# generalizable-neural-performer/bodyfitting

Measured on NVIDIA B200. Metric: fitted frames/s (SMPL-X, 8 views, 100 iters), higher is better.
Workload: dtype fp32

## Files before the change

bodyfitting_b200/csrc/bf_api.cu:

```cuda
#include <math.h>
#include <stdarg.h>
#include <string.h>
#include <stddef.h>
#include <stdlib.h>

#include "bf_common.cuh"
#include "bf_pose.cuh"
#include "bf_skin.cuh"
#include "bf_loss.cuh"
#include "bf_gmm.cuh"
#include "bf_frame.cuh"
#include "bf_ops.cuh"
#include "bf_grid.cuh"
#include "bf_mask.cuh"
#include "../../include/bodyfit_b200_ops.h"
#include "bf_blend_tc.cuh"
#include "bf_blend_tc2.cuh"
#include "bf_pack.cuh"
#include "bf_model_build.cuh"

static thread_local char g_err[512] = "";

void bf_set_error(const char* fmt, ...) {
    va_list ap;
    va_start(ap, fmt);
    vsnprintf(g_err, sizeof(g_err), fmt, ap);
    va_end(ap);
}

static int check_model(const BfModel* m, const BfFrames* f) {
    BF_REQUIRE(m && f, "null model / frames");
    BF_REQUIRE(m->J > 0 && m->J <= BF_MAXJ, "J out of range");
    BF_REQUIRE(m->NS > 0 && m->NS <= BF_MAXNS && m->NB <= m->NS, "NS/NB out of range");
    BF_REQUIRE(m->face == 0 || (m->face == 1 && m->is_smplx), "face parameters apply to SMPL-X only");
    BF_REQUIRE(m->NP == theta_layout(*m).np && theta_layout(m->is_smplx, m->NB).np <= BF_MAXNP && m->NP <= BF_THETA_SMEM,
               "NP does not match theta layout");
    BF_REQUIRE(m->Kp % 16 == 0 && m->Kp >= m->P + m->NS + 1, "Kp must be a multiple of 16 covering P+NS+1");
    BF_REQUIRE(m->P == (m->J - 1) * 9, "P != 9(J-1)");
    BF_REQUIRE(m->parents && m->lvl_ptr && m->lvl_j && m->child_ptr && m->child_idx, "kinematic tree tables missing");
    BF_REQUIRE(f->B > 0, "B <= 0");
    BF_REQUIRE(f->theta, "theta is null");
    return BF_OK;
}

static int check_vset(const BfVSet* vs, const BfFrames* f) {
    BF_REQUIRE(vs->Bm && vs->ell_j && vs->ell_w, "vertex set tables missing");
    BF_REQUIRE(vs->n > 0 && vs->n_pad % 32 == 0 && vs->n_pad >= vs->n && vs->ldn == 3 * vs->n_pad, "bad vertex set padding");
    BF_REQUIRE(f->ld_v >= 3 * vs->n, "ld_v < 3n");
    BF_REQUIRE(vs->K_out <= BF_MAXK, "too many output joints");
    return BF_OK;
}

extern "C" {

int bf_abi_version(void) { return BF_ABI_VERSION; }
int bf_sizeof(int which) {
    switch (which) {
        case 0: return (int)sizeof(BfVSet);
        case 1: return (int)sizeof(BfModel);
        case 2: return (int)sizeof(BfFrames);
        case 3: return (int)sizeof(BfGrid);
        case 4: return (int)sizeof(BfSmpld);
        case 5: return (int)sizeof(BfMask);
        default: return -1;
    }
}
const char* bf_last_error(void) { return g_err; }

int bf_check_device(void) {
    int dev = 0;
    cudaDeviceProp p;
    if (cudaGetDevice(&dev) != cudaSuccess || cudaGetDeviceProperties(&p, dev) != cudaSuccess) {
        bf_set_error("bf_check_device: no CUDA device");
        return BF_ECUDA;
    }
    if (p.major != 10) {
        bf_set_error("bf_check_device: device %s is sm_%d%d; this library is sm_100a only (no fallback)", p.name, p.major, p.minor);
        return BF_EARCH;
    }
    return BF_OK;
}

int bf_pose_forward(const BfModel* m, const BfFrames* f, void* stream) {
    BF_NVTX();
    int rc = check_model(m, f); if (rc) return rc;
    BF_REQUIRE(f->pf && f->A && f->Jtr, "pf/A/Jtr is null");
    const int wpb = 4;
    const dim3 grid((f->B + wpb - 1) / wpb), block(32 * wpb);
    k_pose_fwd<<<grid, block, wpb * sizeof(PoseSmem), (cudaStream_t)stream>>>(*m, *f);
    BF_LAUNCH_CHECK();
    return BF_OK;
}

int bf_skin_forward(const BfModel* m, const BfFrames* f, int use_full, void* stream) {
    BF_NVTX();
    int rc = check_model(m, f); if (rc) return rc;
    const BfVSet* vs = use_full ? &m->full : &m->act;
    rc = check_vset(vs, f); if (rc) return rc;
    BF_REQUIRE(f->pf && f->A && f->verts, "pf/A/verts is null");
    if (bf_tc_ready_fwd(vs, f)) {
        float* vp = f->vposed ? f->vposed : f->verts;
        rc = bf_blend_forward_tc(m, vs, f, vp, (cudaStream_t)stream); if (rc) return rc;
        rc = bf_launch_skin_frame(0, m, vs, f, vp, f->verts, nullptr, nullptr, 0, (f->flags & BF_F_WORLD) ? 1 : 0, 0, (cudaStream_t)stream);
        if (rc != 1) return rc;
        return bf_launch_skin_rows(0, vs, m->J, f->A, vp, f->verts, nullptr, nullptr, f->B, f->ld_v, 0,
                                   (f->flags & BF_F_WORLD) ? f->theta : nullptr, m->NP, f->constant_scale, (cudaStream_t)stream);
    }
    const dim3 grid(vs->n_pad / SK_TV, (f->B + SK_TB - 1) / SK_TB), block(256);
    k_skin_fwd<<<grid, block, 0, (cudaStream_t)stream>>>(*vs, m->J, m->Kp, f->pf, f->A, f->verts, f->vposed, f->B, f->ld_v,
                                                           (f->flags & BF_F_WORLD) ? f->theta : nullptr, m->NP, f->constant_scale);
    BF_LAUNCH_CHECK();
    return BF_OK;
}

int bf_blend_forward(const BfModel* m, const BfFrames* f, int use_full, void* stream) {
    BF_NVTX();
    int rc = check_model(m, f); if (rc) return rc;
    const BfVSet* vs = use_full ? &m->full : &m->act;
    rc = check_vset(vs, f); if (rc) return rc;
    BF_REQUIRE(f->vposed, "vposed is null");
    BF_REQUIRE((f->flags & BF_F_TC) && vs->Bt_hi && vs->Bt_lo && f->pf_hi && f->pf_lo, "bf_blend_forward needs the tensor-core operands (BF_F_TC)");
    return bf_blend_forward_tc(m, vs, f, f->vposed, (cudaStream_t)stream);
}

int bf_joints_forward(const BfModel* m, const BfFrames* f, int use_full, void* stream) {
    BF_NVTX();
    int rc = check_model(m, f); if (rc) return rc;
    const BfVSet* vs = use_full ? &m->full : &m->act;
    rc = check_vset(vs, f); if (rc) return rc;
    BF_REQUIRE(f->joints && f->Jtr && f->verts, "joints/Jtr/verts is null");
    k_joints_fwd<<<f->B, 160, 0, (cudaStream_t)stream>>>(*m, *vs, *f);
    BF_LAUNCH_CHECK();
    return BF_OK;
}

int bf_joints_backward(const BfModel* m, const BfFrames* f, int use_full, int accumulate_dverts, void* stream) {
    BF_NVTX();
    int rc = check_model(m, f); if (rc) return rc;
    const BfVSet* vs = use_full ? &m->full : &m->act;
    rc = check_vset(vs, f); if (rc) return rc;
    BF_REQUIRE(f->dJtr && f->dverts, "dJtr/dverts is null");
    k_joints_bwd<<<f->B, 256, 0, (cudaStream_t)stream>>>(*m, *vs, *f, accumulate_dverts);
    BF_LAUNCH_CHECK();
    return BF_OK;
}

int bf_keypoint_loss(const BfModel* m, const BfFrames* f, int use_full, void* stream) {
    BF_NVTX();
    int rc = check_model(m, f); if (rc) return rc;
    const BfVSet* vs = use_full ? &m->full : &m->act;
    rc = check_vset(vs, f); if (rc) return rc;
    BF_REQUIRE(f->kp && f->cams && f->loss && f->grad && f->dJtr && f->dverts && f->verts && f->Jtr, "loss buffers missing");
    BF_REQUIRE(f->Nv > 0 && f->Nv <= BF_MAXVIEWS, "Nv out of range");
    BF_REQUIRE(m->K_used <= vs->K_out, "K_used > K_out");
    const int threads = use_full ? 256 : 160;
    k_keypoint_loss<<<f->B, threads, 0, (cudaStream_t)stream>>>(*m, *vs, *f);
    BF_LAUNCH_CHECK();
    return BF_OK;
}

struct SideStream { cudaStream_t main = nullptr; cudaStream_t s = nullptr; cudaEvent_t fork = nullptr, join = nullptr; int dev = -1, slot = 0; };
static SideStream* side_stream(cudaStream_t main_s, int slot = 0) {
    static SideStream table[512];
    static int used = 0;
    int dev = 0;
    if (cudaGetDevice(&dev) != cudaSuccess) return nullptr;
    std::lock_guard<std::mutex> lk(g_bf_mu);
    for (int i = 0; i < used; ++i)
        if (table[i].dev == dev && table[i].main == main_s && table[i].slot == slot) return &table[i];
    if (used >= 512) return nullptr;
    SideStream* ss = &table[used];
    if (cudaStreamCreateWithFlags(&ss->s, cudaStreamNonBlocking) != cudaSuccess) return nullptr;
// ... 128 lines not shown
        rc = bf_gemm_forward_tc(x_hi, x_lo, m->gmm_bt_hi, m->gmm_bt_lo, f->B, GM_KG, ny, ny / 3, Y, ny, s); if (rc) return rc;
        k_gmm_select<<<(f->B + 3) / 4, 128, 0, s>>>(*m, f->theta + 7, m->NP, nb, f->B, Y, ny, wp, f->gmm_grad, f->gmm_loss);
        BF_LAUNCH_CHECK();
        return BF_OK;
    }
    return launch_gmm(m, f->theta + 7, m->NP, theta_layout(m->is_smplx).nbody, f->B, f->w_pose * f->w_pose,
                      f->gmm_grad, f->gmm_loss, (cudaStream_t)stream);
}

int bf_op_project(const float* pts, const float* R, const float* t, const float* K, float* uv, int B, int N, int nb, void* stream) {
    BF_REQUIRE(pts && R && t && K && uv && B > 0 && N > 0 && (nb == 1 || nb == B), "bad arguments");
    k_project_fwd<<<(B * N + 255) / 256, 256, 0, (cudaStream_t)stream>>>(pts, R, t, K, uv, B, N, nb);
    BF_LAUNCH_CHECK();
    return BF_OK;
}
int bf_op_project_backward(const float* pts, const float* R, const float* t, const float* K, const float* duv, float* dpts,
                           int B, int N, int nb, void* stream) {
    BF_REQUIRE(pts && R && t && K && duv && dpts && B > 0 && N > 0 && (nb == 1 || nb == B), "bad arguments");
    k_project_bwd<<<(B * N + 255) / 256, 256, 0, (cudaStream_t)stream>>>(pts, R, t, K, duv, dpts, B, N, nb);
    BF_LAUNCH_CHECK();
    return BF_OK;
}
int bf_op_gmof(const float* x, float* y, float sigma, int64_t n, void* stream) {
    BF_REQUIRE(x && y && n > 0, "bad arguments");
    k_gmof_fwd<<<(unsigned)((n + 255) / 256), 256, 0, (cudaStream_t)stream>>>(x, y, sigma, (size_t)n);
    BF_LAUNCH_CHECK();
    return BF_OK;
}
int bf_op_gmof_backward(const float* x, const float* dy, float* dx, float sigma, int64_t n, void* stream) {
    BF_REQUIRE(x && dy && dx && n > 0, "bad arguments");
    k_gmof_bwd<<<(unsigned)((n + 255) / 256), 256, 0, (cudaStream_t)stream>>>(x, dy, dx, sigma, (size_t)n);
    BF_LAUNCH_CHECK();
    return BF_OK;
}
int bf_op_reprojection(const float* cord, const float* gt, const float* w, float coef, float sigma, int N, float* out,
                       float* dcord, void* stream) {
    BF_REQUIRE(cord && gt && w && out && dcord && N > 0, "bad arguments");
    k_reproj<<<1, 256, 0, (cudaStream_t)stream>>>(cord, gt, w, coef, sigma, N, out, dcord);
    BF_LAUNCH_CHECK();
    return BF_OK;
}
int bf_op_keypoints_world(const float* joints, const float* kp, const float* cams, int B, int K, int Nv, float coef,
                          float sigma, float* loss_bk, float* dJ, void* stream) {
    BF_REQUIRE(joints && kp && cams && loss_bk && dJ && B > 0 && K > 0 && Nv > 0, "bad arguments");
    k_kp_world<<<(B * K + 127) / 128, 128, 0, (cudaStream_t)stream>>>(joints, kp, cams, B, K, Nv, coef, sigma, loss_bk, dJ);
    BF_LAUNCH_CHECK();
    return BF_OK;
}
int bf_op_angle_prior(const float* pose, int B, int D, float* out, float* dout, void* stream) {
    BF_REQUIRE(pose && out && dout && B > 0 && D >= 56, "bad arguments (pose needs >= 56 columns)");
    k_angle_prior<<<(B * 4 + 127) / 128, 128, 0, (cudaStream_t)stream>>>(pose, B, D, out, dout);
    BF_LAUNCH_CHECK();
    return BF_OK;
}
int bf_op_gmm_pose(const BfModel* m, const float* pose, int ld, int nvalid, int B, float weight, float* grad, float* loss,
                   void* stream) {
    BF_REQUIRE(m && nvalid > 0 && nvalid <= 69 && ld >= nvalid, "bad arguments");
    return launch_gmm(m, pose, ld, nvalid, B, weight, grad, loss, (cudaStream_t)stream);
}

int bf_pose_backward(const BfModel* m, const BfFrames* f, int flags, void* stream) {
    BF_NVTX();
    int rc = check_model(m, f); if (rc) return rc;
    BF_REQUIRE(f->dA && f->dJtr && f->dpf && f->grad && f->loss, "pose backward buffers missing");
    if (flags & 1) BF_REQUIRE(f->gmm_grad && f->gmm_loss, "gmm_grad / gmm_loss missing (run bf_gmm_prior first)");
    if (flags & 8) BF_REQUIRE((flags & 2) && f->pf && f->A && f->Jtr, "flag 8 needs the Adam step and the forward buffers");
    if (flags & 2) BF_REQUIRE(f->adam_m && f->adam_v, "Adam state missing");
    const double t = (double)(f->iter + 1);
    const double bc1 = 1.0 - pow(f->beta1, t);
    const double bc2 = 1.0 - pow(f->beta2, t);
    AdamArgs ad;
    ad.step_ts = (float)(f->lr_ts / bc1);
    ad.step_lr = (float)(f->lr / bc1);
    ad.bc2_sqrt = (float)sqrt(bc2);
    ad.beta2 = (float)f->beta2;
    ad.om_beta1 = (float)(1.0 - f->beta1);
    ad.om_beta2 = (float)(1.0 - f->beta2);
    ad.eps = (float)f->eps;
    static int wpb = 0;
    if (!wpb) { const char* e = getenv("BODYFIT_POSE_WPB"); wpb = e ? atoi(e) : 2; if (wpb < 1 || wpb > 4) wpb = 2; }
    const dim3 grid((f->B + wpb - 1) / wpb), block(32 * wpb);
    BfFrames g = *f;
    if (!bf_bwd_two_cta(m, f)) g.dpf2 = nullptr;
    k_pose_bwd<<<grid, block, wpb * sizeof(PoseSmemBwd), (cudaStream_t)stream>>>(*m, g, flags, ad);
    BF_LAUNCH_CHECK();
    return BF_OK;
}

int bf_lbs_forward(const BfModel* m, const BfFrames* f, void* stream) {
    BF_NVTX();
    int rc = bf_pose_forward(m, f, stream); if (rc) return rc;
    const BfVSet* vs = &m->full;
    if (f->joints && bf_tc_ready_fwd(vs, f) && f->verts && f->Jtr) {
        rc = check_vset(vs, f); if (rc) return rc;
        float* vp = f->vposed ? f->vposed : f->verts;
        rc = bf_blend_forward_tc(m, vs, f, vp, (cudaStream_t)stream); if (rc) return rc;
        rc = bf_launch_skin_frame(0, m, vs, f, vp, f->verts, nullptr, nullptr, 0, (f->flags & BF_F_WORLD) ? 1 : 0, 1, (cudaStream_t)stream);
        if (rc == 2) return BF_OK;
        if (rc == BF_OK) return bf_joints_forward(m, f, 1, stream);
        if (rc != 1) return rc;
        rc = bf_launch_skin_rows(0, vs, m->J, f->A, vp, f->verts, nullptr, nullptr, f->B, f->ld_v, 0,
                                 (f->flags & BF_F_WORLD) ? f->theta : nullptr, m->NP, f->constant_scale, (cudaStream_t)stream);
        if (rc) return rc;
        return bf_joints_forward(m, f, 1, stream);
    }
    rc = bf_skin_forward(m, f, 1, stream); if (rc) return rc;
    if (f->joints) rc = bf_joints_forward(m, f, 1, stream);
    return rc;
}

int bf_lbs_backward(const BfModel* m, const BfFrames* f, void* stream) {
    BF_NVTX();
    int rc = bf_joints_backward(m, f, 1, 1, stream); if (rc) return rc;
    rc = bf_skin_backward(m, f, 1, stream); if (rc) return rc;
    return bf_pose_backward(m, f, 0, stream);
}

static size_t bf_frame_smem(const BfModel* m, const BfVSet* vs, int Nv, int tma) {
    return sizeof(float) * (size_t)frame_smem_layout(m->K_used, Nv, m->J, vs->ldn, vs->lmax, tma).total;
}
static bool bf_frame_use_tma(const BfModel* m, const BfVSet* vs, const BfFrames* f) {
    static int env = -1;
    if (env < 0) { const char* e = getenv("BODYFIT_FRAME_TMA"); env = e ? atoi(e) : 1; }
    return env != 0 && (m->K_used * f->Nv) % 4 == 0 && ((uintptr_t)f->kp & 15) == 0 && ((uintptr_t)f->A & 15) == 0 &&
           ((uintptr_t)f->vposed & 15) == 0 && bf_frame_smem(m, vs, f->Nv, 1) <= 48 * 1024;
}

int bf_frame_loss_backward(const BfModel* m, const BfFrames* f, void* stream) {
    BF_NVTX();
    int rc = check_model(m, f); if (rc) return rc;
    const BfVSet* vs = &m->act;
    rc = check_vset(vs, f); if (rc) return rc;
    const int skin_here = (f->flags & BF_F_SKIN_FUSED) ? 1 : 0;
    BF_REQUIRE(f->kp && f->cams && f->loss && f->grad && f->dJtr && (skin_here || f->verts) && f->vposed && f->Jtr && f->A && f->dA,
               "fused loss/backward buffers missing");
    BF_REQUIRE(vs->lv_n && vs->lv_vid && vs->lt_ptr && vs->lt_k && vs->lt_w && vs->lj_ptr && vs->lj_vid && vs->lj_w && vs->lmax > 0 &&
               vs->n_rows > 0, "live-vertex lists of the active set missing");
    BF_REQUIRE(f->ld_v % 4 == 0 && vs->ldn % 4 == 0, "ld_v / ldn must be multiples of 4 floats");
    BF_REQUIRE(f->dvp_hi || f->dvp, "dvp (or its 3xTF32 split) missing");
    BF_REQUIRE(f->Nv > 0 && f->Nv <= BF_MAXVIEWS, "Nv out of range");
    BF_REQUIRE(vs->jv_ptr && vs->jv_vid && vs->jv_w && vs->jv_nz, "joint->vertex lists missing");
    const bool tma = bf_frame_use_tma(m, vs, f);
    const size_t smem = bf_frame_smem(m, vs, f->Nv, tma);
    BF_REQUIRE(smem <= 48 * 1024, "active vertex set too large for the fused per-frame kernel");
    BfFrames g = *f;
    if (!bf_tc_ready_bwd(vs, f)) { g.dvp_hi = nullptr; g.dvp_lo = nullptr; }
    static int nt_env = -1;
    if (nt_env < 0) { const char* e = getenv("BODYFIT_FRAME_THREADS"); const int v = e ? atoi(e) : 0; nt_env = (v == 256 || v == 224 || v == 160) ? v : 0; }
    const int nt = nt_env ? nt_env : (f->B >= 2048 ? 160 : 224);
    const cudaStream_t s_ = (cudaStream_t)stream;
    if (tma && nt == 160) {
        const size_t smem2 = bf_frame_smem(m, vs, f->Nv, 2);
        static bool carve[BF_MAXDEV] = {false};
        const int dev = bf_cur_dev();
        {
            std::lock_guard<std::mutex> lk(g_bf_mu);
            if (!carve[dev]) {
                cudaFuncSetAttribute(k_frame_loss_bwd<2, 160>, cudaFuncAttributePreferredSharedMemoryCarveout, 100);
                cudaGetLastError();
                carve[dev] = true;
            }
        }
        k_frame_loss_bwd<2, 160><<<f->B, 160, smem2, s_>>>(*m, *vs, g, skin_here);
    } else if (tma) {
        if (nt == 256) k_frame_loss_bwd<1, 256><<<f->B, 256, smem, s_>>>(*m, *vs, g, skin_here);
        else k_frame_loss_bwd<1, 224><<<f->B, 224, smem, s_>>>(*m, *vs, g, skin_here);
    } else {
// ... 648 lines not shown
```

bodyfitting_b200/csrc/bf_pose.cuh:

```cuda
#pragma once
#include "bf_common.cuh"
#include "bf_pack.cuh"

struct PoseSmem {
    float th[BF_THETA_SMEM];
    float sh[BF_MAXNS];
    float fp[BF_MAXJ * 3];
    float R[BF_MAXJ * 9];
    float Jr[BF_MAXJ * 3];
    float GR[BF_MAXJ * 9];
    float Gt[BF_MAXJ * 3];
};
static_assert((BF_THETA_SMEM + BF_MAXNS) % 4 == 0 && offsetof(PoseSmem, fp) % 16 == 0, "PoseSmem::fp must be 16-byte aligned");
static_assert(BF_THETA_SMEM >= BF_MAXNP - 9 + BF_MAXNS, "PoseSmem::th must hold the longest face-parameter row");
struct __align__(16) PoseSmemBwd {
    PoseSmem f;
    float dGR[BF_MAXJ * 9];
    uint64_t bar;
};
static_assert(sizeof(PoseSmemBwd) <= 8464, "k_pose_bwd: 13 CTAs of 2 frames per SM need <= 8464 bytes per frame");
static_assert(BF_THETA_SMEM <= 128 && 128 + BF_MAXJ * 3 <= BF_MAXJ * 9, "gradient row / d(rest joints) must fit into PoseSmem::R");

__device__ __forceinline__ void pose_forward_from_smem(const BfModel& m, PoseSmem& S, int lane);

__device__ __forceinline__ void pose_forward_warp(const BfModel& m, const float* __restrict__ theta_row,
                                                  PoseSmem& S, int lane) {
    const int np = theta_layout(m).np;
    for (int i = lane; i < np; i += 32) S.th[i] = theta_row[i];
    __syncwarp();
    pose_forward_from_smem(m, S, lane);
}

__device__ __forceinline__ void pose_forward_from_smem(const BfModel& m, PoseSmem& S, int lane) {
    const ThetaLayout L = theta_layout(m);
    const int J = m.J;
    for (int i = lane; i < 3 * J; i += 32) {
        float v = 0.f;
        if (i < 3) v = S.th[4 + i];
        else if (i < 3 + L.nbody) v = S.th[7 + (i - 3)];
        else if (m.is_smplx) {
            if (i < 69) v = m.face ? S.th[L.off_jaw + (i - 66)] : 0.f;
            else if (i < 72) v = S.th[L.off_leye + (i - 69)];
            else if (i < 75) v = S.th[L.off_reye + (i - 72)];
            else if (i < 120) {
                const int c0 = i - 75;
#pragma unroll
                for (int c = 0; c < 6; ++c) v += S.th[L.off_lh + c] * __ldg(m.hand_l + c * 45 + c0);
            } else {
                const int c0 = i - 120;
#pragma unroll
                for (int c = 0; c < 6; ++c) v += S.th[L.off_rh + c] * __ldg(m.hand_r + c * 45 + c0);
            }
        }
        S.fp[i] = v + __ldg(m.pose_mean + i);
    }
    for (int l = lane; l < m.NS; l += 32) S.sh[l] = (l < m.NB) ? S.th[L.off_betas + l] : m.face ? S.th[L.off_expr + (l - m.NB)] : 0.f;
    __syncwarp();
    for (int j = lane; j < J; j += 32) {
        float R[9];
        rodrigues_fwd(S.fp[3 * j], S.fp[3 * j + 1], S.fp[3 * j + 2], R);
#pragma unroll
        for (int e = 0; e < 9; ++e) S.R[j * 9 + e] = R[e];
        if (m.NB == 10 && (m.NS & 3) == 0) {
            float sh[10];
#pragma unroll
            for (int l = 0; l < 10; ++l) sh[l] = S.sh[l];
#pragma unroll
            for (int c = 0; c < 3; ++c) {
                const float* jd = m.Jd + (j * 3 + c) * m.NS;
                const float4 a = __ldg(reinterpret_cast<const float4*>(jd)), q = __ldg(reinterpret_cast<const float4*>(jd) + 1);
                const float2 r = __ldg(reinterpret_cast<const float2*>(jd) + 4);
                float acc = 0.f;
                acc += a.x * sh[0]; acc += a.y * sh[1]; acc += a.z * sh[2]; acc += a.w * sh[3];
                acc += q.x * sh[4]; acc += q.y * sh[5]; acc += q.z * sh[6]; acc += q.w * sh[7];
                acc += r.x * sh[8]; acc += r.y * sh[9];
                if (m.face)
                    for (int l = 10; l < m.NS; ++l) acc += __ldg(jd + l) * S.sh[l];
                S.Jr[j * 3 + c] = __ldg(m.Jt + j * 3 + c) + acc;
            }
        } else {
#pragma unroll
            for (int c = 0; c < 3; ++c) {
                float acc = 0.f;
                const float* jd = m.Jd + (j * 3 + c) * m.NS;
                const int nl = m.face ? m.NS : m.NB;
                for (int l = 0; l < nl; ++l) acc += __ldg(jd + l) * S.sh[l];
                S.Jr[j * 3 + c] = __ldg(m.Jt + j * 3 + c) + acc;
            }
        }
    }
    __syncwarp();
    for (int lev = 0; lev <= m.max_depth; ++lev) {
        for (int idx = __ldg(m.lvl_ptr + lev) + lane; idx < __ldg(m.lvl_ptr + lev + 1); idx += 32) {
            const int j = __ldg(m.lvl_j + idx);
            if (lev == 0) {
#pragma unroll
                for (int e = 0; e < 9; ++e) S.GR[j * 9 + e] = S.R[j * 9 + e];
#pragma unroll
                for (int c = 0; c < 3; ++c) S.Gt[j * 3 + c] = S.Jr[j * 3 + c];
            } else {
                const int p = __ldg(m.parents + j);
                float rel[3], G[9];
#pragma unroll
                for (int c = 0; c < 3; ++c) rel[c] = S.Jr[j * 3 + c] - S.Jr[p * 3 + c];
                mat3_mul(&S.GR[p * 9], &S.R[j * 9], G);
#pragma unroll
                for (int e = 0; e < 9; ++e) S.GR[j * 9 + e] = G[e];
#pragma unroll
                for (int r = 0; r < 3; ++r)
                    S.Gt[j * 3 + r] = S.GR[p * 9 + r * 3 + 0] * rel[0] + S.GR[p * 9 + r * 3 + 1] * rel[1] +
                                      S.GR[p * 9 + r * 3 + 2] * rel[2] + S.Gt[p * 3 + r];
            }
        }
        __syncwarp();
    }
}

__device__ __forceinline__ void pose_write_outputs(const BfModel& m, const BfFrames& f, PoseSmem& S, int b, int lane, int mask_par) {
    const int J = m.J;
    if (f.fwd_state) {
        float* st = f.fwd_state + (size_t)b * 24 * J;
        for (int i = lane; i < 3 * J; i += 32) { st[i] = S.fp[i]; st[12 * J + i] = S.Jr[i]; }
        for (int i = lane; i < 9 * J; i += 32) { st[3 * J + i] = S.R[i]; st[15 * J + i] = S.GR[i]; }
    }
    float* pf = f.pf + (size_t)b * m.Kp;
    const bool tc_only = (f.flags & BF_F_TC) && f.pf_hi && f.pf_lo;
    for (int i = lane; i < m.Kp; i += 32) {
        float v = 0.f;
        if (i < m.P) {
            const int e = i % 9;
            v = S.R[9 + i] - ((e == 0 || e == 4 || e == 8) ? 1.0f : 0.0f);
        } else if (i < m.P + m.NS) v = S.sh[i - m.P];
        else if (i == m.P + m.NS) v = 1.0f;
        if (!tc_only) pf[i] = v;
        if (f.pf_hi) {
            float hi, lo;
            split_tf32(v, hi, lo);
            f.pf_hi[(size_t)b * m.Kp + i] = hi;
            f.pf_lo[(size_t)b * m.Kp + i] = lo;
        }
    }
    for (int j = lane; j < J; j += 32) {
        float4* Aj = reinterpret_cast<float4*>(f.A + ((size_t)b * J + j) * 12);
#pragma unroll
        for (int r = 0; r < 3; ++r) {
            const float g0 = S.GR[j * 9 + r * 3], g1 = S.GR[j * 9 + r * 3 + 1], g2 = S.GR[j * 9 + r * 3 + 2];
            const float4 row = make_float4(g0, g1, g2, S.Gt[j * 3 + r] - (g0 * S.Jr[j * 3] + g1 * S.Jr[j * 3 + 1] + g2 * S.Jr[j * 3 + 2]));
            Aj[r] = row;
            f.Jtr[((size_t)b * J + j) * 3 + r] = S.Gt[j * 3 + r];
        }
    }
    if (f.full_pose)
        for (int i = lane; i < 3 * J; i += 32) f.full_pose[(size_t)b * 3 * J + i] = S.fp[i];
    if (lane == 0 && f.yaw) {
        int row = 0;
        if (m.is_smplx) {
            float rel[9], t[9];
#pragma unroll
            for (int e = 0; e < 9; ++e) rel[e] = S.R[12 * 9 + e];
            const int chain[4] = {9, 6, 3, 0};
#pragma unroll
            for (int q = 0; q < 4; ++q) {
                mat3_mul(&S.R[chain[q] * 9], rel, t);
#pragma unroll
                for (int e = 0; e < 9; ++e) rel[e] = t[e];
            }
            const float sy = sqrtf(rel[0] * rel[0] + rel[3] * rel[3]);
            const float ang = atan2f(-rel[6], sy);
            float y = rintf(fminf((-ang * 180.0f) / 3.14159265358979323846f, 39.0f));
            int yi = (int)y;
            if (yi < 0) yi = (yi < -39) ? 78 : (39 - yi);
            row = yi;
        }
        f.yaw[b] = row;
        if (f.blk_mask && m.act.lv_blk)
            atomicOr(f.blk_mask + (size_t)mask_par * ((f.B + 127) >> 7) + (b >> 7), __ldg(m.act.lv_blk + (m.act.n_rows > 1 ? row : 0)));
    }
}

__global__ void __launch_bounds__(128) k_pose_fwd(BfModel m, BfFrames f) {
    extern __shared__ __align__(16) unsigned char smem_raw[];
    PoseSmem* all = reinterpret_cast<PoseSmem*>(smem_raw);
    const int warp = threadIdx.x >> 5, lane = threadIdx.x & 31;
    const int b = blockIdx.x * (blockDim.x >> 5) + warp;
    if (b >= f.B) return;
    PoseSmem& S = all[warp];
    pose_forward_warp(m, f.theta + (size_t)b * m.NP, S, lane);
    pose_write_outputs(m, f, S, b, lane, f.iter & 1);
}

struct AdamArgs { float step_ts, step_lr, bc2_sqrt, beta2, om_beta1, om_beta2, eps; };

__global__ void __launch_bounds__(128, 7) k_pose_bwd(BfModel m, BfFrames f, int flags, AdamArgs ad) {
    extern __shared__ __align__(16) unsigned char smem_raw[];
    PoseSmemBwd* all = reinterpret_cast<PoseSmemBwd*>(smem_raw);
    const int warp = threadIdx.x >> 5, lane = threadIdx.x & 31;
    const int b = blockIdx.x * (blockDim.x >> 5) + warp;
    if (b >= f.B) return;
    PoseSmemBwd& W = all[warp];
    PoseSmem& S = W.f;
    float* const drel = S.Gt;
    float* const dfp = S.fp;
    const int J = m.J;
    const ThetaLayout L = theta_layout(m);
    const bool use_bulk = f.fwd_state && J == BF_MAXJ && ((uintptr_t)f.fwd_state & 15) == 0;
    if (use_bulk) {
        if (lane == 0) {
            tc::mbar_init(&W.bar, 1);
            asm volatile("fence.mbarrier_init.release.cluster;" ::: "memory");
            asm volatile("fence.proxy.async.shared::cta;" ::: "memory");
            const float* st = f.fwd_state + (size_t)b * 24 * J;
            tc::mbar_expect_tx(&W.bar, (uint32_t)(96 * J));
            tc::bulk_g2s(S.fp, st, (uint32_t)(96 * J), &W.bar);
        }
    }
    float4 dA_r[2][3];
    float dJ_r[2][3];
#pragma unroll
    for (int s = 0; s < 2; ++s) {
        const int j = lane + 32 * s;
        if (j < J) {
            const float4* dAj = reinterpret_cast<const float4*>(f.dA + ((size_t)b * J + j) * 12);
            const float* dJj = f.dJtr + ((size_t)b * J + j) * 3;
            dA_r[s][0] = dAj[0]; dA_r[s][1] = dAj[1]; dA_r[s][2] = dAj[2];
            dJ_r[s][0] = dJj[0]; dJ_r[s][1] = dJj[1]; dJ_r[s][2] = dJj[2];
        }
    }
    float am_r[4], av_r[4], gg_r[3];
    if (flags & 2) {
#pragma unroll
        for (int s = 0; s < 4; ++s) {
            const int i = lane + 32 * s;
            if (i < m.NP) { am_r[s] = f.adam_m[(size_t)b * m.NP + i]; av_r[s] = f.adam_v[(size_t)b * m.NP + i]; }
        }
    }
    if (flags & 1) {
#pragma unroll
        for (int s = 0; s < 3; ++s) {
            const int i = lane + 32 * s;
            gg_r[s] = i < L.nbody ? f.gmm_grad[(size_t)b * BF_GMM_D + i] : 0.f;
        }
    }
    float* const g = S.R;
    float* const dJr_s = S.R + 128;
    const float g_ts = (lane < 4 && (flags & 4)) ? f.grad[(size_t)b * m.NP + lane] : 0.f;
    if (f.fwd_state) {
        for (int i = lane; i < L.np; i += 32) S.th[i] = f.theta[(size_t)b * m.NP + i];
        if (use_bulk) {
            __syncwarp();
            int spins = 0;
            while (!tc::mbar_try(&W.bar, 0)) { if (++spins > (1 << 26)) __trap(); }
        } else {
            const float* st = f.fwd_state + (size_t)b * 24 * J;
            for (int i = lane; i < 3 * J; i += 32) { S.fp[i] = st[i]; S.Jr[i] = st[12 * J + i]; }
            for (int i = lane; i < 9 * J; i += 32) { S.R[i] = st[3 * J + i]; S.GR[i] = st[15 * J + i]; }
        }
        __syncwarp();
    } else {
        pose_forward_warp(m, f.theta + (size_t)b * m.NP, S, lane);
    }

    float dJr_r[2][3];
#pragma unroll
    for (int s = 0; s < 2; ++s) {
        const int j = lane + 32 * s;
        if (j >= J) break;
        const float dAj[12] = {dA_r[s][0].x, dA_r[s][0].y, dA_r[s][0].z, dA_r[s][0].w, dA_r[s][1].x, dA_r[s][1].y, dA_r[s][1].z, dA_r[s][1].w,
                               dA_r[s][2].x, dA_r[s][2].y, dA_r[s][2].z, dA_r[s][2].w};
        float dAt[3];
#pragma unroll
        for (int r = 0; r < 3; ++r) {
            dAt[r] = dAj[r * 4 + 3];
            S.Gt[j * 3 + r] = dJ_r[s][r] + dAt[r];
#pragma unroll
            for (int c = 0; c < 3; ++c) W.dGR[j * 9 + r * 3 + c] = dAj[r * 4 + c] - dAt[r] * S.Jr[j * 3 + c];
        }
#pragma unroll
        for (int c = 0; c < 3; ++c)
            dJr_r[s][c] = -(S.GR[j * 9 + 0 * 3 + c] * dAt[0] + S.GR[j * 9 + 1 * 3 + c] * dAt[1] +
                            S.GR[j * 9 + 2 * 3 + c] * dAt[2]);
    }
    __syncwarp();
    for (int lev = m.max_depth - 1; lev >= 0; --lev) {
        for (int idx = __ldg(m.lvl_ptr + lev) + lane; idx < __ldg(m.lvl_ptr + lev + 1); idx += 32) {
            const int j = __ldg(m.lvl_j + idx);
            const int c0 = __ldg(m.child_ptr + j), c1 = __ldg(m.child_ptr + j + 1);
            if (c0 == c1) continue;
            float aR[9], aT[3], pj[3];
#pragma unroll
            for (int e = 0; e < 9; ++e) aR[e] = W.dGR[j * 9 + e];
#pragma unroll
            for (int c = 0; c < 3; ++c) { aT[c] = S.Gt[j * 3 + c]; pj[c] = S.Jr[j * 3 + c]; }
            for (int q = c0; q < c1; ++q) {
                const int ch = __ldg(m.child_idx + q);
                float rel[3], Rc[9];
#pragma unroll
                for (int c = 0; c < 3; ++c) rel[c] = S.Jr[ch * 3 + c] - pj[c];
#pragma unroll
                for (int e = 0; e < 9; ++e) Rc[e] = S.R[ch * 9 + e];
#pragma unroll
                for (int r = 0; r < 3; ++r) {
                    const float g0 = W.dGR[ch * 9 + r * 3], g1 = W.dGR[ch * 9 + r * 3 + 1], g2 = W.dGR[ch * 9 + r * 3 + 2];
                    const float gt = S.Gt[ch * 3 + r];
#pragma unroll
                    for (int c = 0; c < 3; ++c)
                        aR[r * 3 + c] += g0 * Rc[c * 3] + g1 * Rc[c * 3 + 1] + g2 * Rc[c * 3 + 2] + gt * rel[c];
                    aT[r] += gt;
                }
            }
#pragma unroll
            for (int e = 0; e < 9; ++e) W.dGR[j * 9 + e] = aR[e];
#pragma unroll
            for (int c = 0; c < 3; ++c) S.Gt[j * 3 + c] = aT[c];
        }
        __syncwarp();
    }
    for (int j = lane; j < J; j += 32) {
        float dR[9], dr[3];
        if (j == 0) {
#pragma unroll
            for (int e = 0; e < 9; ++e) dR[e] = W.dGR[e];
#pragma unroll
            for (int c = 0; c < 3; ++c) dr[c] = S.Gt[c];
        } else {
            const int p = __ldg(m.parents + j);
#pragma unroll
            for (int r = 0; r < 3; ++r) {
#pragma unroll
                for (int c = 0; c < 3; ++c)
                    dR[r * 3 + c] = S.GR[p * 9 + 0 * 3 + r] * W.dGR[j * 9 + 0 * 3 + c] +
                                    S.GR[p * 9 + 1 * 3 + r] * W.dGR[j * 9 + 1 * 3 + c] +
                                    S.GR[p * 9 + 2 * 3 + r] * W.dGR[j * 9 + 2 * 3 + c];
                dr[r] = S.GR[p * 9 + 0 * 3 + r] * S.Gt[j * 3 + 0] + S.GR[p * 9 + 1 * 3 + r] * S.Gt[j * 3 + 1] +
                        S.GR[p * 9 + 2 * 3 + r] * S.Gt[j * 3 + 2];
            }
            const float* dpf = f.dpf + (size_t)b * m.Kp + (j - 1) * 9;
            if (f.dpf2) {
                const float* dq = f.dpf2 + (size_t)b * m.Kp + (j - 1) * 9;
#pragma unroll
                for (int e = 0; e < 9; ++e) dR[e] += dpf[e] + dq[e];
            } else {
#pragma unroll
                for (int e = 0; e < 9; ++e) dR[e] += dpf[e];
            }
        }
#pragma unroll
        for (int c = 0; c < 3; ++c) drel[j * 3 + c] = dr[c];
        float g[3];
        rodrigues_bwd(S.fp[3 * j], S.fp[3 * j + 1], S.fp[3 * j + 2], dR, g);
#pragma unroll
        for (int c = 0; c < 3; ++c) dfp[j * 3 + c] = g[c];
    }
    __syncwarp();
#pragma unroll
    for (int s = 0; s < 2; ++s) {
        const int j = lane + 32 * s;
        if (j >= J) break;
        float acc[3] = {drel[j * 3], drel[j * 3 + 1], drel[j * 3 + 2]};
        const int c0 = __ldg(m.child_ptr + j), c1 = __ldg(m.child_ptr + j + 1);
        for (int q = c0; q < c1; ++q) {
            const int ch = __ldg(m.child_idx + q);
#pragma unroll
            for (int c = 0; c < 3; ++c) acc[c] -= drel[ch * 3 + c];
        }
#pragma unroll
        for (int c = 0; c < 3; ++c) dJr_s[j * 3 + c] = dJr_r[s][c] + acc[c];
    }
    if (lane < 4) g[lane] = g_ts;
    __syncwarp();

    {
        const int l = lane % m.NB, part = lane / m.NB;
        const int nparts = 3 * m.NB <= 32 ? 3 : 2 * m.NB <= 32 ? 2 : 1;
        const int nq = 3 * J, per = (nq + nparts - 1) / nparts;
        float acc = 0.f;
        if (part < nparts) {
            const int q1 = min(nq, (part + 1) * per);
#pragma unroll 11
            for (int q = part * per; q < q1; ++q) acc += __ldg(m.Jd + q * m.NS + l) * dJr_s[q];
        }
        const float a1s = __shfl_sync(0xffffffffu, acc, (lane + m.NB) & 31);
        const float a2s = __shfl_sync(0xffffffffu, acc, (lane + 2 * m.NB) & 31);
        const float a1 = nparts > 1 ? a1s : 0.f;
        const float a2 = nparts > 2 ? a2s : 0.f;
        if (lane < m.NB) {
            float dsh = f.dpf[(size_t)b * m.Kp + m.P + lane];
            if (f.dpf2) dsh += f.dpf2[(size_t)b * m.Kp + m.P + lane];
            g[L.off_betas + lane] = dsh + ((acc + a1) + a2);
        }
    }
    if (m.face) {
        const int ne = m.NS - m.NB;
        if (ne > 0) {
            const int e = lane % ne, part = lane / ne;
            const int nparts = 3 * ne <= 32 ? 3 : 2 * ne <= 32 ? 2 : 1;
            const int nq = 3 * J, per = (nq + nparts - 1) / nparts;
            float acc = 0.f;
            if (part < nparts) {
                const int q1 = min(nq, (part + 1) * per);
                for (int q = part * per; q < q1; ++q) acc += __ldg(m.Jd + q * m.NS + m.NB + e) * dJr_s[q];
            }
            const float a1s = __shfl_sync(0xffffffffu, acc, (lane + ne) & 31);
            const float a2s = __shfl_sync(0xffffffffu, acc, (lane + 2 * ne) & 31);
            const float a1 = nparts > 1 ? a1s : 0.f;
            const float a2 = nparts > 2 ? a2s : 0.f;
            if (lane < ne) {
                float dsh = f.dpf[(size_t)b * m.Kp + m.P + m.NB + lane];
                if (f.dpf2) dsh += f.dpf2[(size_t)b * m.Kp + m.P + m.NB + lane];
                g[L.off_expr + lane] = dsh + ((acc + a1) + a2);
            }
        }
        if (lane < 3) g[L.off_jaw + lane] = dfp[66 + lane];
    }
    for (int i = lane; i < 3 + L.nbody; i += 32) g[4 + i] = dfp[i];
    if (m.is_smplx) {
        if (lane < 3) { g[L.off_leye + lane] = dfp[69 + lane]; g[L.off_reye + lane] = dfp[72 + lane]; }
        if (lane < 12) {
            const int c = lane % 6;
            const float* comp = (lane < 6 ? m.hand_l : m.hand_r) + c * 45;
            const float* d = dfp + (lane < 6 ? 75 : 120);
            float acc = 0.f;
#pragma unroll 15
            for (int i = 0; i < 45; ++i) acc += __ldg(comp + i) * d[i];
            g[(lane < 6 ? L.off_lh : L.off_rh) + c] = acc;
        }
    }
    __syncwarp();

    float total = (flags & 4) ? f.loss[b] : 0.f;
    if (flags & 1) {
#pragma unroll
        for (int s = 0; s < 3; ++s) {
            const int i = lane + 32 * s;
            if (i < L.nbody) g[7 + i] += gg_r[s];
        }
        const float pose_l = f.gmm_loss[b];
        __syncwarp();
        float temp_l = 0.f;
        if (f.tgrad) {
            for (int i = lane; i < m.NP; i += 32) g[i] += f.tgrad[(size_t)b * m.NP + i];
            temp_l = f.tloss[b];
            __syncwarp();
        }
        float ang = 0.f;
        if (lane < 4) {
            const int idx = (lane == 0) ? 52 : (lane == 1) ? 55 : (lane == 2) ? 9 : 12;
            const float sg = (lane == 0) ? 1.0f : -1.0f;
            const float e = expf(S.th[7 + idx] * sg);
            ang = e * e;
            g[7 + idx] += f.w_angle * f.w_angle * 2.0f * ang * sg;
        }
        const float angle_l = f.w_angle * f.w_angle * warp_sum(ang);
        float sq = 0.f;
        if (lane < m.NB) {
            const float be = S.th[L.off_betas + lane];
            sq = be * be;
            g[L.off_betas + lane] += f.w_shape * f.w_shape * 2.0f * be;
        }
        float shape_l = f.w_shape * f.w_shape * warp_sum(sq);
        if (m.face) {
            float eq = 0.f;
            if (lane < m.NS - m.NB) {
                const float ps = S.th[L.off_expr + lane];
                eq = ps * ps;
                g[L.off_expr + lane] += f.w_expr * f.w_expr * 2.0f * ps;
            }
            shape_l += f.w_expr * f.w_expr * warp_sum(eq);
        }
        if (lane == 0 && f.loss_terms) {
            f.loss_terms[b * 4 + 0] = total;
            f.loss_terms[b * 4 + 1] = pose_l;
            f.loss_terms[b * 4 + 2] = angle_l;
            f.loss_terms[b * 4 + 3] = shape_l;
        }
        total += pose_l + angle_l + shape_l + temp_l;
    }
    if (lane == 0) {
        f.loss[b] = total;
        if (f.trace) f.trace[(size_t)f.iter * f.B + b] = total;
    }
    __syncwarp();
    for (int i = lane; i < m.NP; i += 32) f.grad[(size_t)b * m.NP + i] = g[i];
    if (flags & 2) {
        float* th = f.theta + (size_t)b * m.NP;
        float* am = f.adam_m + (size_t)b * m.NP;
        float* av = f.adam_v + (size_t)b * m.NP;
#pragma unroll
        for (int s = 0; s < 4; ++s) {
            const int i = lane + 32 * s;
            if (i >= m.NP) break;
            const float gi = g[i];
            float mi = am_r[s], vi = av_r[s];
            mi = mi + (gi - mi) * ad.om_beta1;
            vi = vi * ad.beta2 + ad.om_beta2 * gi * gi;
            const float denom = sqrtf(vi) / ad.bc2_sqrt + ad.eps;
            const float step = (i < 4) ? ad.step_ts : ad.step_lr;
            const float tn = S.th[i] + (-step) * mi / denom;
            th[i] = tn;
            am[i] = mi; av[i] = vi;
            S.th[i] = tn;
        }
        if ((flags & 16) && f.halo_buf && (b == 0 || b + 1 == f.B)) {
            __syncwarp();
            const uint32_t tick = *reinterpret_cast<const uint32_t*>(f.halo_buf + BF_HALO_EPOCH) + (uint32_t)f.iter + 1u;
            if (b == 0 && f.halo_peer_prev) halo_push_row(S.th, m.NP, f.halo_peer_prev, BF_HALO_NEXT, tick, lane);
            if (b + 1 == f.B && f.halo_peer_next) halo_push_row(S.th, m.NP, f.halo_peer_next, BF_HALO_PREV, tick, lane);
        }
        if (flags & 8) {
            __syncwarp();
            pose_forward_from_smem(m, S, lane);
            pose_write_outputs(m, f, S, b, lane, (f.iter + 1) & 1);
        }
    }
}
```

Measured before the change: 204,000.

## Shrink pose backward smem: recompute rotations, alias dGR, stage topology in smem

Stops storing per-joint rotation matrices R in the forward state, shrinking the bulk copy. The backward pass now recomputes them with Rodrigues per tree level into a small scratch area, and dGR is aliased onto S.R, so per-frame shared memory drops and launch bounds rise from 7 to 8 blocks. The kinematic topology tables (levels, parents, children) are staged once per CTA as bytes in shared memory instead of repeated __ldg reads, and the theta/Adam loads move later. The cost is extra Rodrigues computation and an added block-wide sync in both kernels.

```diff
diff --git a/bodyfitting_b200/csrc/bf_api.cu b/bodyfitting_b200/csrc/bf_api.cu
--- a/bodyfitting_b200/csrc/bf_api.cu
+++ b/bodyfitting_b200/csrc/bf_api.cu
@@ -87,7 +87,7 @@
     BF_REQUIRE(f->pf && f->A && f->Jtr, "pf/A/Jtr is null");
     const int wpb = 4;
     const dim3 grid((f->B + wpb - 1) / wpb), block(32 * wpb);
-    k_pose_fwd<<<grid, block, wpb * sizeof(PoseSmem), (cudaStream_t)stream>>>(*m, *f);
+    k_pose_fwd<<<grid, block, sizeof(PoseTopo) + wpb * sizeof(PoseSmem), (cudaStream_t)stream>>>(*m, *f);
     BF_LAUNCH_CHECK();
     return BF_OK;
 }
@@ -382,7 +382,7 @@
     const dim3 grid((f->B + wpb - 1) / wpb), block(32 * wpb);
     BfFrames g = *f;
     if (!bf_bwd_two_cta(m, f)) g.dpf2 = nullptr;
-    k_pose_bwd<<<grid, block, wpb * sizeof(PoseSmemBwd), (cudaStream_t)stream>>>(*m, g, flags, ad);
+    k_pose_bwd<<<grid, block, sizeof(PoseTopo) + wpb * sizeof(PoseSmemBwd), (cudaStream_t)stream>>>(*m, g, flags, ad);
     BF_LAUNCH_CHECK();
     return BF_OK;
 }
diff --git a/bodyfitting_b200/csrc/bf_pose.cuh b/bodyfitting_b200/csrc/bf_pose.cuh
--- a/bodyfitting_b200/csrc/bf_pose.cuh
+++ b/bodyfitting_b200/csrc/bf_pose.cuh
@@ -6,32 +6,60 @@
     float th[BF_THETA_SMEM];
     float sh[BF_MAXNS];
     float fp[BF_MAXJ * 3];
-    float R[BF_MAXJ * 9];
     float Jr[BF_MAXJ * 3];
     float GR[BF_MAXJ * 9];
     float Gt[BF_MAXJ * 3];
+    float R[BF_MAXJ * 9];
 };
 static_assert((BF_THETA_SMEM + BF_MAXNS) % 4 == 0 && offsetof(PoseSmem, fp) % 16 == 0, "PoseSmem::fp must be 16-byte aligned");
 static_assert(BF_THETA_SMEM >= BF_MAXNP - 9 + BF_MAXNS, "PoseSmem::th must hold the longest face-parameter row");
+#define BF_POSE_STATE_COPY(J) ((15 * (J) + 3) & ~3)
+static_assert(offsetof(PoseSmem, Gt) - offsetof(PoseSmem, fp) == 15 * BF_MAXJ * sizeof(float) &&
+              BF_POSE_STATE_COPY(BF_MAXJ) - 15 * BF_MAXJ <= 3 * BF_MAXJ, "the bulk copy of the state row must end inside PoseSmem::Gt");
 struct __align__(16) PoseSmemBwd {
     PoseSmem f;
-    float dGR[BF_MAXJ * 9];
     uint64_t bar;
 };
-static_assert(sizeof(PoseSmemBwd) <= 8464, "k_pose_bwd: 13 CTAs of 2 frames per SM need <= 8464 bytes per frame");
+static_assert(sizeof(PoseSmemBwd) <= 6480, "k_pose_bwd: 16 CTAs of 2 frames per SM need <= 6480 bytes per frame");
 static_assert(BF_THETA_SMEM <= 128 && 128 + BF_MAXJ * 3 <= BF_MAXJ * 9, "gradient row / d(rest joints) must fit into PoseSmem::R");
 
-__device__ __forceinline__ void pose_forward_from_smem(const BfModel& m, PoseSmem& S, int lane);
-
-__device__ __forceinline__ void pose_forward_warp(const BfModel& m, const float* __restrict__ theta_row,
+struct __align__(16) PoseTopo {
+    unsigned char lvl_ptr[BF_MAXJ + 1];
+    unsigned char lvl_j[BF_MAXJ];
+    unsigned char parents[BF_MAXJ];
+    unsigned char child_ptr[BF_MAXJ + 1];
+    unsigned char child_idx[BF_MAXJ];
+    unsigned char lvl_pos[BF_MAXJ];
+};
+static_assert(sizeof(PoseTopo) == 336 && BF_MAXJ < 255, "PoseTopo: byte entries, 16-byte multiple");
+
+__device__ __forceinline__ void pose_topo_stage(const BfModel& m, PoseTopo& T) {
+    const int J = m.J;
+    for (int i = threadIdx.x; i <= J; i += blockDim.x) {
+        if (i <= m.max_depth + 1) T.lvl_ptr[i] = (unsigned char)__ldg(m.lvl_ptr + i);
+        T.child_ptr[i] = (unsigned char)__ldg(m.child_ptr + i);
+        if (i < J) {
+            const int lj = __ldg(m.lvl_j + i);
+            T.lvl_j[i] = (unsigned char)lj;
+            T.lvl_pos[lj] = (unsigned char)i;
+            T.parents[i] = (unsigned char)__ldg(m.parents + i);
+            T.child_idx[i] = (unsigned char)__ldg(m.child_idx + i);
+        }
+    }
+    __syncthreads();
+}
+
+__device__ __forceinline__ void pose_forward_from_smem(const BfModel& m, const PoseTopo& T, PoseSmem& S, int lane);
+
+__device__ __forceinline__ void pose_forward_warp(const BfModel& m, const PoseTopo& T, const float* __restrict__ theta_row,
                                                   PoseSmem& S, int lane) {
     const int np = theta_layout(m).np;
     for (int i = lane; i < np; i += 32) S.th[i] = theta_row[i];
     __syncwarp();
-    pose_forward_from_smem(m, S, lane);
+    pose_forward_from_smem(m, T, S, lane);
 }
 
-__device__ __forceinline__ void pose_forward_from_smem(const BfModel& m, PoseSmem& S, int lane) {
+__device__ __forceinline__ void pose_forward_from_smem(const BfModel& m, const PoseTopo& T, PoseSmem& S, int lane) {
     const ThetaLayout L = theta_layout(m);
     const int J = m.J;
     for (int i = lane; i < 3 * J; i += 32) {
@@ -91,15 +119,16 @@
     }
     __syncwarp();
     for (int lev = 0; lev <= m.max_depth; ++lev) {
-        for (int idx = __ldg(m.lvl_ptr + lev) + lane; idx < __ldg(m.lvl_ptr + lev + 1); idx += 32) {
-            const int j = __ldg(m.lvl_j + idx);
+        const int i1 = T.lvl_ptr[lev + 1];
+        for (int idx = T.lvl_ptr[lev] + lane; idx < i1; idx += 32) {
+            const int j = T.lvl_j[idx];
             if (lev == 0) {
 #pragma unroll
                 for (int e = 0; e < 9; ++e) S.GR[j * 9 + e] = S.R[j * 9 + e];
 #pragma unroll
                 for (int c = 0; c < 3; ++c) S.Gt[j * 3 + c] = S.Jr[j * 3 + c];
             } else {
-                const int p = __ldg(m.parents + j);
+                const int p = T.parents[j];
                 float rel[3], G[9];
 #pragma unroll
                 for (int c = 0; c < 3; ++c) rel[c] = S.Jr[j * 3 + c] - S.Jr[p * 3 + c];
@@ -120,8 +149,9 @@
     const int J = m.J;
     if (f.fwd_state) {
         float* st = f.fwd_state + (size_t)b * 24 * J;
-        for (int i = lane; i < 3 * J; i += 32) { st[i] = S.fp[i]; st[12 * J + i] = S.Jr[i]; }
-        for (int i = lane; i < 9 * J; i += 32) { st[3 * J + i] = S.R[i]; st[15 * J + i] = S.GR[i]; }
+        for (int i = lane; i < 3 * J; i += 32) { st[i] = S.fp[i]; st[3 * J + i] = S.Jr[i]; }
+        for (int i = lane; i < 9 * J; i += 32) st[6 * J + i] = S.GR[i];
+        if (lane < BF_POSE_STATE_COPY(J) - 15 * J) st[15 * J + lane] = 0.f;
     }
     float* pf = f.pf + (size_t)b * m.Kp;
     const bool tc_only = (f.flags & BF_F_TC) && f.pf_hi && f.pf_lo;
@@ -180,40 +210,45 @@
 
 __global__ void __launch_bounds__(128) k_pose_fwd(BfModel m, BfFrames f) {
     extern __shared__ __align__(16) unsigned char smem_raw[];
-    PoseSmem* all = reinterpret_cast<PoseSmem*>(smem_raw);
+    PoseTopo& T = *reinterpret_cast<PoseTopo*>(smem_raw);
+    PoseSmem* all = reinterpret_cast<PoseSmem*>(smem_raw + sizeof(PoseTopo));
     const int warp = threadIdx.x >> 5, lane = threadIdx.x & 31;
     const int b = blockIdx.x * (blockDim.x >> 5) + warp;
+    pose_topo_stage(m, T);
     if (b >= f.B) return;
     PoseSmem& S = all[warp];
-    pose_forward_warp(m, f.theta + (size_t)b * m.NP, S, lane);
+    pose_forward_warp(m, T, f.theta + (size_t)b * m.NP, S, lane);
     pose_write_outputs(m, f, S, b, lane, f.iter & 1);
 }
 
 struct AdamArgs { float step_ts, step_lr, bc2_sqrt, beta2, om_beta1, om_beta2, eps; };
 
-__global__ void __launch_bounds__(128, 7) k_pose_bwd(BfModel m, BfFrames f, int flags, AdamArgs ad) {
+__global__ void __launch_bounds__(128, 8) k_pose_bwd(BfModel m, BfFrames f, int flags, AdamArgs ad) {
     extern __shared__ __align__(16) unsigned char smem_raw[];
-    PoseSmemBwd* all = reinterpret_cast<PoseSmemBwd*>(smem_raw);
+    PoseTopo& T = *reinterpret_cast<PoseTopo*>(smem_raw);
+    PoseSmemBwd* all = reinterpret_cast<PoseSmemBwd*>(smem_raw + sizeof(PoseTopo));
     const int warp = threadIdx.x >> 5, lane = threadIdx.x & 31;
     const int b = blockIdx.x * (blockDim.x >> 5) + warp;
-    if (b >= f.B) return;
     PoseSmemBwd& W = all[warp];
     PoseSmem& S = W.f;
+    float* const dGR = S.R;
     float* const drel = S.Gt;
     float* const dfp = S.fp;
     const int J = m.J;
     const ThetaLayout L = theta_layout(m);
     const bool use_bulk = f.fwd_state && J == BF_MAXJ && ((uintptr_t)f.fwd_state & 15) == 0;
-    if (use_bulk) {
-        if (lane == 0) {
-            tc::mbar_init(&W.bar, 1);
-            asm volatile("fence.mbarrier_init.release.cluster;" ::: "memory");
-            asm volatile("fence.proxy.async.shared::cta;" ::: "memory");
-            const float* st = f.fwd_state + (size_t)b * 24 * J;
-            tc::mbar_expect_tx(&W.bar, (uint32_t)(96 * J));
-            tc::bulk_g2s(S.fp, st, (uint32_t)(96 * J), &W.bar);
-        }
-    }
+    if (use_bulk && b < f.B && lane == 0) {
+        tc::mbar_init(&W.bar, 1);
+        asm volatile("fence.mbarrier_init.release.cluster;" ::: "memory");
+        asm volatile("fence.proxy.async.shared::cta;" ::: "memory");
+        const float* st = f.fwd_state + (size_t)b * 24 * J;
+        const uint32_t bytes = (uint32_t)(4 * BF_POSE_STATE_COPY(J));
+        tc::mbar_expect_tx(&W.bar, bytes);
+        tc::bulk_g2s(S.fp, st, bytes, &W.bar);
+    }
+    pose_topo_stage(m, T);
+    if (b >= f.B) return;
+    if (!f.fwd_state) pose_forward_warp(m, T, f.theta + (size_t)b * m.NP, S, lane);
     float4 dA_r[2][3];
     float dJ_r[2][3];
 #pragma unroll
@@ -226,38 +261,19 @@
             dJ_r[s][0] = dJj[0]; dJ_r[s][1] = dJj[1]; dJ_r[s][2] = dJj[2];
         }
     }
-    float am_r[4], av_r[4], gg_r[3];
-    if (flags & 2) {
-#pragma unroll
-        for (int s = 0; s < 4; ++s) {
-            const int i = lane + 32 * s;
-            if (i < m.NP) { am_r[s] = f.adam_m[(size_t)b * m.NP + i]; av_r[s] = f.adam_v[(size_t)b * m.NP + i]; }
-        }
-    }
-    if (flags & 1) {
-#pragma unroll
-        for (int s = 0; s < 3; ++s) {
-            const int i = lane + 32 * s;
-            gg_r[s] = i < L.nbody ? f.gmm_grad[(size_t)b * BF_GMM_D + i] : 0.f;
-        }
-    }
-    float* const g = S.R;
-    float* const dJr_s = S.R + 128;
-    const float g_ts = (lane < 4 && (flags & 4)) ? f.grad[(size_t)b * m.NP + lane] : 0.f;
     if (f.fwd_state) {
-        for (int i = lane; i < L.np; i += 32) S.th[i] = f.theta[(size_t)b * m.NP + i];
         if (use_bulk) {
             __syncwarp();
             int spins = 0;
             while (!tc::mbar_try(&W.bar, 0)) { if (++spins > (1 << 26)) __trap(); }
         } else {
             const float* st = f.fwd_state + (size_t)b * 24 * J;
-            for (int i = lane; i < 3 * J; i += 32) { S.fp[i] = st[i]; S.Jr[i] = st[12 * J + i]; }
-            for (int i = lane; i < 9 * J; i += 32) { S.R[i] = st[3 * J + i]; S.GR[i] = st[15 * J + i]; }
+#pragma unroll 1
+            for (int i = lane; i < 3 * J; i += 32) { S.fp[i] = st[i]; S.Jr[i] = st[3 * J + i]; }
+#pragma unroll 1
+            for (int i = lane; i < 9 * J; i += 32) S.GR[i] = st[6 * J + i];
         }
         __syncwarp();
-    } else {
-        pose_forward_warp(m, f.theta + (size_t)b * m.NP, S, lane);
     }
 
     float dJr_r[2][3];
@@ -273,7 +289,7 @@
             dAt[r] = dAj[r * 4 + 3];
             S.Gt[j * 3 + r] = dJ_r[s][r] + dAt[r];
 #pragma unroll
-            for (int c = 0; c < 3; ++c) W.dGR[j * 9 + r * 3 + c] = dAj[r * 4 + c] - dAt[r] * S.Jr[j * 3 + c];
+            for (int c = 0; c < 3; ++c) dGR[j * 9 + r * 3 + c] = dAj[r * 4 + c] - dAt[r] * S.Jr[j * 3 + c];
         }
 #pragma unroll
         for (int c = 0; c < 3; ++c)
@@ -281,26 +297,44 @@
                             S.GR[j * 9 + 2 * 3 + c] * dAt[2]);
     }
     __syncwarp();
+    float* const Rs = S.th;
+    constexpr int kRs = (BF_THETA_SMEM + BF_MAXNS) / 9;
+    static_assert(offsetof(PoseSmem, sh) == BF_THETA_SMEM * sizeof(float), "th and sh are one scratch block");
     for (int lev = m.max_depth - 1; lev >= 0; --lev) {
-        for (int idx = __ldg(m.lvl_ptr + lev) + lane; idx < __ldg(m.lvl_ptr + lev + 1); idx += 32) {
-            const int j = __ldg(m.lvl_j + idx);
-            const int c0 = __ldg(m.child_ptr + j), c1 = __ldg(m.child_ptr + j + 1);
+        const int i1 = T.lvl_ptr[lev + 1];
+        const int nch = T.lvl_ptr[lev + 2] - i1;
+        if (lane < nch && lane < kRs) {
+            const int ch = T.lvl_j[i1 + lane];
+            float R[9];
+            rodrigues_fwd(S.fp[ch * 3], S.fp[ch * 3 + 1], S.fp[ch * 3 + 2], R);
+#pragma unroll
+            for (int e = 0; e < 9; ++e) Rs[lane * 9 + e] = R[e];
+        }
+        __syncwarp();
+        for (int idx = T.lvl_ptr[lev] + lane; idx < i1; idx += 32) {
+            const int j = T.lvl_j[idx];
+            const int c0 = T.child_ptr[j], c1 = T.child_ptr[j + 1];
             if (c0 == c1) continue;
             float aR[9], aT[3], pj[3];
 #pragma unroll
-            for (int e = 0; e < 9; ++e) aR[e] = W.dGR[j * 9 + e];
+            for (int e = 0; e < 9; ++e) aR[e] = dGR[j * 9 + e];
 #pragma unroll
             for (int c = 0; c < 3; ++c) { aT[c] = S.Gt[j * 3 + c]; pj[c] = S.Jr[j * 3 + c]; }
             for (int q = c0; q < c1; ++q) {
-                const int ch = __ldg(m.child_idx + q);
+                const int ch = T.child_idx[q];
                 float rel[3], Rc[9];
 #pragma unroll
                 for (int c = 0; c < 3; ++c) rel[c] = S.Jr[ch * 3 + c] - pj[c];
-#pragma unroll
-                for (int e = 0; e < 9; ++e) Rc[e] = S.R[ch * 9 + e];
+                const int pos = T.lvl_pos[ch] - i1;
+                if (pos < kRs) {
+#pragma unroll
+                    for (int e = 0; e < 9; ++e) Rc[e] = Rs[pos * 9 + e];
+                } else {
+                    rodrigues_fwd(S.fp[ch * 3], S.fp[ch * 3 + 1], S.fp[ch * 3 + 2], Rc);
+                }
 #pragma unroll
                 for (int r = 0; r < 3; ++r) {
-                    const float g0 = W.dGR[ch * 9 + r * 3], g1 = W.dGR[ch * 9 + r * 3 + 1], g2 = W.dGR[ch * 9 + r * 3 + 2];
+                    const float g0 = dGR[ch * 9 + r * 3], g1 = dGR[ch * 9 + r * 3 + 1], g2 = dGR[ch * 9 + r * 3 + 2];
                     const float gt = S.Gt[ch * 3 + r];
 #pragma unroll
                     for (int c = 0; c < 3; ++c)
@@ -309,28 +343,47 @@
                 }
             }
 #pragma unroll
-            for (int e = 0; e < 9; ++e) W.dGR[j * 9 + e] = aR[e];
+            for (int e = 0; e < 9; ++e) dGR[j * 9 + e] = aR[e];
 #pragma unroll
             for (int c = 0; c < 3; ++c) S.Gt[j * 3 + c] = aT[c];
         }
         __syncwarp();
     }
+    for (int i = lane; i < m.NP; i += 32) S.th[i] = f.theta[(size_t)b * m.NP + i];
+    float am_r[4], av_r[4], gg_r[3];
+    if (flags & 2) {
+#pragma unroll
+        for (int s = 0; s < 4; ++s) {
+            const int i = lane + 32 * s;
+            if (i < m.NP) { am_r[s] = f.adam_m[(size_t)b * m.NP + i]; av_r[s] = f.adam_v[(size_t)b * m.NP + i]; }
+        }
+    }
+    if (flags & 1) {
+#pragma unroll
+        for (int s = 0; s < 3; ++s) {
+            const int i = lane + 32 * s;
+            gg_r[s] = i < L.nbody ? f.gmm_grad[(size_t)b * BF_GMM_D + i] : 0.f;
+        }
+    }
+    float* const g = S.R;
+    float* const dJr_s = S.R + 128;
+    const float g_ts = (lane < 4 && (flags & 4)) ? f.grad[(size_t)b * m.NP + lane] : 0.f;
     for (int j = lane; j < J; j += 32) {
         float dR[9], dr[3];
         if (j == 0) {
 #pragma unroll
-            for (int e = 0; e < 9; ++e) dR[e] = W.dGR[e];
+            for (int e = 0; e < 9; ++e) dR[e] = dGR[e];
 #pragma unroll
             for (int c = 0; c < 3; ++c) dr[c] = S.Gt[c];
         } else {
-            const int p = __ldg(m.parents + j);
+            const int p = T.parents[j];
 #pragma unroll
             for (int r = 0; r < 3; ++r) {
 #pragma unroll
                 for (int c = 0; c < 3; ++c)
-                    dR[r * 3 + c] = S.GR[p * 9 + 0 * 3 + r] * W.dGR[j * 9 + 0 * 3 + c] +
-                                    S.GR[p * 9 + 1 * 3 + r] * W.dGR[j * 9 + 1 * 3 + c] +
-                                    S.GR[p * 9 + 2 * 3 + r] * W.dGR[j * 9 + 2 * 3 + c];
+                    dR[r * 3 + c] = S.GR[p * 9 + 0 * 3 + r] * dGR[j * 9 + 0 * 3 + c] +
+                                    S.GR[p * 9 + 1 * 3 + r] * dGR[j * 9 + 1 * 3 + c] +
+                                    S.GR[p * 9 + 2 * 3 + r] * dGR[j * 9 + 2 * 3 + c];
                 dr[r] = S.GR[p * 9 + 0 * 3 + r] * S.Gt[j * 3 + 0] + S.GR[p * 9 + 1 * 3 + r] * S.Gt[j * 3 + 1] +
                         S.GR[p * 9 + 2 * 3 + r] * S.Gt[j * 3 + 2];
             }
@@ -357,9 +410,9 @@
         const int j = lane + 32 * s;
         if (j >= J) break;
         float acc[3] = {drel[j * 3], drel[j * 3 + 1], drel[j * 3 + 2]};
-        const int c0 = __ldg(m.child_ptr + j), c1 = __ldg(m.child_ptr + j + 1);
+        const int c0 = T.child_ptr[j], c1 = T.child_ptr[j + 1];
         for (int q = c0; q < c1; ++q) {
-            const int ch = __ldg(m.child_idx + q);
+            const int ch = T.child_idx[q];
 #pragma unroll
             for (int c = 0; c < 3; ++c) acc[c] -= drel[ch * 3 + c];
         }
@@ -508,7 +561,7 @@
         }
         if (flags & 8) {
             __syncwarp();
-            pose_forward_from_smem(m, S, lane);
+            pose_forward_from_smem(m, T, S, lane);
             pose_write_outputs(m, f, S, b, lane, (f.iter + 1) & 1);
         }
     }
```

New measurement: 209,900 (median of 6 runs). 2.9% higher.
